# skit-ai/N-Best-ASR-Transformer

Measured on AMD Instinct MI355X. Metric: utterances/sec fine-tune (bert-base, seq128, n_best=5), higher is better.
Workload: dtype bf16

## Files before the change

include/nbest_hip.h:

```cpp
#ifndef NBEST_HIP_H
#define NBEST_HIP_H

#include <stddef.h>
#include <stdint.h>

#ifdef __cplusplus
extern "C" {
#endif

#define NBEST_ABI_VERSION 1

enum { NBEST_OK = 0, NBEST_ERR_ARG = -1, NBEST_ERR_SHAPE = -2, NBEST_ERR_DTYPE = -3, NBEST_ERR_ALIGN = -4,
       NBEST_ERR_LAUNCH = -5, NBEST_ERR_WORKSPACE = -6 };
enum { NBEST_F32 = 0, NBEST_BF16 = 1 };

typedef void* nbest_stream_t;

int nbest_version(void);
int nbest_last_error(char* buf, size_t n);

int nbest_embed_ln_fwd(const int64_t* ids, const int64_t* seg, const int64_t* pos, const void* word,
                       const void* type, const void* ptab, const float* gamma, const float* beta, void* out,
                       float* stats, int64_t M, int H, float eps, int dtype, float drop_p, uint64_t seed,
                       uint32_t drop_stream, nbest_stream_t stream);
// ... 176 lines not shown
} nbest_tensor_desc;
int nbest_bertadam_chunk(void);
int nbest_bertadam_step(float* p, float* g, float* m, float* v, void* p_lowp, const nbest_tensor_desc* descs,
                        int n_tensors, int n_blocks, float lr_mult, float b1, float b2, float eps,
                        float max_grad_norm, void* ws, size_t ws_bytes, nbest_stream_t stream);
int nbest_bertadam_norms(const float* g, const nbest_tensor_desc* descs, int n_tensors, int n_blocks, int blk_lo, int blk_hi,
                         float* partial, nbest_stream_t stream);
int nbest_bertadam_update(float* p, const float* g, float* m, float* v, void* p_lowp, const nbest_tensor_desc* descs,
                          int n_tensors, int n_blocks, int blk_lo, int blk_hi, const float* partial, float* coef,
                          float lr_mult, float b1, float b2, float eps, float max_grad_norm, nbest_stream_t stream);
enum { NBEST_ADAM_L2 = 0, NBEST_ADAMW = 1 };
int nbest_adam_clip_coef(const float* partial, int n_partial, float max_grad_norm, float* clip, nbest_stream_t stream);
int nbest_adam_update(int mode, float* p, const float* g, float* m, float* v, void* p_lowp, const nbest_tensor_desc* descs,
                      int n_tensors, int n_blocks, int blk_lo, int blk_hi, const float* clip, float lr_mult, float bc1,
                      float bc2_sqrt, double b1, double b2, float eps, nbest_stream_t stream);
int nbest_adam_step(int mode, float* p, float* g, float* m, float* v, void* p_lowp, const nbest_tensor_desc* descs,
                    int n_tensors, int n_blocks, float lr_mult, float bc1, float bc2_sqrt, double b1, double b2, float eps,
                    float max_grad_norm, void* ws, size_t ws_bytes, nbest_stream_t stream);
typedef struct nbest_matrix_desc {
  int64_t offset;
  int32_t rows, cols;
  int32_t tile_start, pad;
} nbest_matrix_desc;
#define NBEST_AMAX_TENSOR_WORDS 1024
int nbest_fp8_amax_fold(void* slots, void* out, int32_t n_tensors, nbest_stream_t stream);
int nbest_quantize_weights_fp8(const float* master, void* w8, void* w8t, const nbest_matrix_desc* descs, int n_matrices,
                               int n_tiles, float* inv_scale, void* ws, size_t ws_bytes, nbest_stream_t stream);
int nbest_transpose_weights(const void* src, void* dst, const nbest_matrix_desc* descs, int n_matrices, int n_tiles,
                            nbest_stream_t stream);
int nbest_pack_bn(int64_t N);
int nbest_pack_bn_fp8(int64_t N, int64_t K);
int nbest_pack_weights_fp8(const void* src, void* dst, const nbest_matrix_desc* descs, int n_matrices, int n_stages, nbest_stream_t stream);
int nbest_pack_weights(const void* src, void* dst, const nbest_matrix_desc* descs, int n_matrices, int n_stages, nbest_stream_t stream);
int nbest_cast_f32_to_bf16(const float* src, void* dst, int64_t n, nbest_stream_t stream);

typedef struct nbest_layer_offsets {
  int64_t wqkv, bqkv, wo, bo, ln1_g, ln1_b, w1, b1, w2, b2, ln2_g, ln2_b;
} nbest_layer_offsets;
typedef struct nbest_encoder_desc {
  int32_t dtype, B, S, H, L, heads, F;
  int32_t vocab, max_pos, n_types;
  float ln_eps, hidden_drop, attn_drop;
  int64_t word_pad_id, pos_pad_id;
  int64_t off_word, off_pos, off_type, off_emb_ln_g, off_emb_ln_b;
  const nbest_layer_offsets* layers_host;
  uint64_t seed;
  uint32_t drop_stream_base;
  int32_t wgrad_events_n;
  void** wgrad_events;
  const void* w8;
  const float* w8_inv_scale;
  const void* w8t;
  const uint32_t* gamax_prev;
  uint32_t* gamax_new;
  int32_t fp8_bwd;
  int32_t pad2;
  const void* wpk;
  const void* wpkt;
  const void* w8p;
  const void* w8tp;
  const int32_t* word_perm;
  const uint32_t* aamax_prev;
  uint32_t* aamax_new;
  int32_t fp8_act;
  int32_t pad4;
  int32_t first_trainable;
// ... 35 lines not shown
```

n-best-asr-transformer_amd/arena.py:

```python
import ctypes as C

import torch

from . import hipabi as hb
from .synth import encoder_param_shapes, head_param_shapes

ALIGN = 64

NO_DECAY = ("bias", "LayerNorm.bias", "LayerNorm.weight")


class Slot:
    __slots__ = ("name", "shape", "offset", "numel")

    def __init__(self, name, shape, offset):
        self.name, self.shape, self.offset = name, tuple(shape), offset
        n = 1
        for s in shape:
            n *= s
        self.numel = n


class ParamArena:
    def __init__(self, cfg, labels, device, compute_dtype=torch.bfloat16):
# ... 71 lines not shown
        self._pdescs = None
        if self.w16 is not None and self.device.type == "cuda":
            self.w16t = torch.zeros(self.total, dtype=torch.bfloat16, device=self.device)
            H, F = cfg.hidden_size, cfg.intermediate_size
            mats = []
            for o in self.layer_offsets:
                mats += [(o.wqkv, 3 * H, H), (o.wo, H, H), (o.w1, F, H), (o.w2, H, F)]
            arr = (hb.MatrixDesc * len(mats))()
            t = 0
            for i, (off, r, c) in enumerate(mats):
                arr[i].offset, arr[i].rows, arr[i].cols, arr[i].tile_start = off, r, c, t
                t += ((r + 63) // 64) * ((c + 63) // 64)
            self._tdescs = (torch.frombuffer(bytearray(bytes(arr)), dtype=torch.uint8).to(self.device), len(mats), t)
            self._pdescs = []
            for transposed in (False, True):
                sel = []
                for off, r, c in mats:
                    n, k = (c, r) if transposed else (r, c)
                    bn = hb.lib().nbest_pack_bn(n)
                    if not (bn > 0 and k % 32 == 0 and n % bn == 0):
                        sel = None
                        break
                    sel.append((off, n, k, bn))
                if sel is None:
                    self._pdescs = None
                    break
                parr = (hb.MatrixDesc * len(sel))()
                t = 0
                for i, (off, n, k, bn) in enumerate(sel):
                    parr[i].offset, parr[i].rows, parr[i].cols, parr[i].tile_start, parr[i].pad = off, n, k, t, bn
                    t += (n // bn) * (k // 32)
                self._pdescs.append((torch.frombuffer(bytearray(bytes(parr)), dtype=torch.uint8).to(self.device), len(sel), t))
            if self._pdescs is not None:
                self.wpk = torch.zeros(self.total, dtype=torch.bfloat16, device=self.device)
                self.wpkt = torch.zeros(self.total, dtype=torch.bfloat16, device=self.device)
        self._descs = None

    def view(self, buf, name):
        s = self.by_name[name]
        return buf[s.offset:s.offset + s.numel].view(s.shape)

    def heads_wb(self):
        R, H = self.labels.n_head_rows, self.cfg.hidden_size
        return self.p[self.off_wh:self.off_wh + R * H].view(R, H), self.p[self.off_bh:self.off_bh + R]

    def heads_grad_wb(self):
        R, H = self.labels.n_head_rows, self.cfg.hidden_size
        return self.g[self.off_wh:self.off_wh + R * H].view(R, H), self.g[self.off_bh:self.off_bh + R]

    @property
    def weights(self):
        return self.w16 if self.w16 is not None else self.p

    def refresh_compute_copy(self):
        if self.w16 is not None:
            hb.cast_bf16(self.p, self.w16)
        self.refresh_transposed()

    def refresh_transposed(self):
        if self.w16t is not None:
            if self.lazy_w16t:
                self.w16t_stale = True
            else:
                self.refresh_w16t()
        if self.w8 is not None:
            d, n, t = self._tdescs
            hb.check(hb.lib().nbest_quantize_weights_fp8(hb.ptr(self.p), hb.ptr(self.w8), hb.ptr(self.w8t), hb.ptr(d), n, t,
                                                         hb.ptr(self.w8_inv_scale), hb.ptr(self._w8_ws), self._w8_ws.numel(),
                                                         hb.stream_ptr()), "quantize_weights_fp8")
            if getattr(self, "w8p", None) is not None:
                for src, dst, (pd, pn, pt) in ((self.w8, self.w8p, self._p8descs[0]), (self.w8t, self.w8tp, self._p8descs[1])):
                    hb.check(hb.lib().nbest_pack_weights_fp8(hb.ptr(src), hb.ptr(dst), hb.ptr(pd), pn, pt, hb.stream_ptr()), "pack_weights_fp8")

    def refresh_w16t(self):
        d, n, t = self._tdescs
        hb.check(hb.lib().nbest_transpose_weights(hb.ptr(self.w16), hb.ptr(self.w16t), hb.ptr(d), n, t, hb.stream_ptr()),
                 "transpose_weights")
        self.w16t_stale = False
        if self.wpk is not None:
            for src, dst, (pd, pn, pt) in ((self.w16, self.wpk, self._pdescs[0]), (self.w16t, self.wpkt, self._pdescs[1])):
                hb.check(hb.lib().nbest_pack_weights(hb.ptr(src), hb.ptr(dst), hb.ptr(pd), pn, pt, hb.stream_ptr()), "pack_weights")

    def enable_fp8_forward(self):
        if self.w16t is None:
            raise RuntimeError("nbest_amd: the fp8 forward needs the bf16 path on a GPU")
        self.wpk = self.wpkt = None
        if self.w8 is None:
            n = self._tdescs[1]
            self.w8 = torch.zeros(self.total, dtype=torch.uint8, device=self.device)
            self.w8t = torch.zeros(self.total, dtype=torch.uint8, device=self.device)
            self.gamax = torch.zeros(n, dtype=torch.int32, device=self.device)
            self.gamax_slots = torch.zeros(n * hb.AMAX_TENSOR_WORDS, dtype=torch.int32, device=self.device)
            self.aamax = torch.zeros(n, dtype=torch.int32, device=self.device)
            self.aamax_slots = torch.zeros(n * hb.AMAX_TENSOR_WORDS, dtype=torch.int32, device=self.device)
            self.w8_inv_scale = torch.ones(n, dtype=torch.float32, device=self.device)
            self._w8_ws = torch.zeros(4 * n + 16, dtype=torch.uint8, device=self.device)
            H, F = self.cfg.hidden_size, self.cfg.intermediate_size
            mats = []
            for o in self.layer_offsets:
                mats += [(o.wqkv, 3 * H, H), (o.wo, H, H), (o.w1, F, H), (o.w2, H, F)]
            self._p8descs = []
            for transposed in (False, True):
                parr = (hb.MatrixDesc * len(mats))()
                t = 0
                for i, (off, r, c) in enumerate(mats):
                    nn, kk = (c, r) if transposed else (r, c)
                    bn = hb.lib().nbest_pack_bn_fp8(nn, kk)
                    if not (bn > 0 and kk % 64 == 0 and nn % bn == 0):
                        parr = None
                        break
                    parr[i].offset, parr[i].rows, parr[i].cols, parr[i].tile_start, parr[i].pad = off, nn, kk, t, bn
                    t += (nn // bn) * (kk // 64)
                if parr is None:
                    self._p8descs = None
# ... 63 lines not shown
```

n-best-asr-transformer_amd/csrc/gemm.hip:

```cpp
#include "common.h"

namespace {

__global__ __launch_bounds__(256) void splitk_reduce_kernel(const float* __restrict__ slab, float* __restrict__ C, int64_t MN,
                                                            int64_t N, int64_t ldc, int splits, int accumulate,
                                                            float* __restrict__ C2, int64_t m_split, int64_t ldc2) {
  for (int64_t i = ((int64_t)blockIdx.x * blockDim.x + threadIdx.x) * 4; i < MN; i += (int64_t)gridDim.x * blockDim.x * 4) {
    f32x4 s = *(const f32x4*)(slab + i);
    for (int z = 1; z < splits; ++z) s += *(const f32x4*)(slab + (int64_t)z * MN + i);
    const int64_t m = i / N, n = i - m * N;
    float* c = (m < m_split) ? C + m * ldc + n : C2 + (m - m_split) * ldc2 + n;
    if (accumulate) s += *(const f32x4*)c;
    *(f32x4*)c = s;
  }
}

int check_epilogue_operands(const nbest_gemm_args* a, int64_t ld_mult, uintptr_t align) {
  const int epi = a->epilogue;
  if (epi == NBEST_EPI_BIAS || epi == NBEST_EPI_BIAS_GELU || epi == NBEST_EPI_BIAS_DROP_RES)
    NB_CHECK(a->bias, NBEST_ERR_ARG, "gemm: epilogue %d needs bias", epi);
  if (epi == NBEST_EPI_BIAS_DROP_RES || epi == NBEST_EPI_RES)
    NB_CHECK(a->R && a->ldr % ld_mult == 0 && ((uintptr_t)a->R & (align - 1)) == 0, NBEST_ERR_ARG, "gemm: epilogue %d needs R", epi);
  if ((epi == NBEST_EPI_BIAS_GELU && a->U) || epi == NBEST_EPI_DGELU)
    NB_CHECK(a->U && a->ldu % ld_mult == 0 && ((uintptr_t)a->U & (align - 1)) == 0, NBEST_ERR_ARG, "gemm: epilogue %d needs U", epi);
// ... 47 lines not shown
  if (a->dtype == NBEST_F32) return (a->colsum_out && a->epilogue != NBEST_EPI_F32_SPLITK) ? nbest_rowred_ws_bytes(a->M, a->N) : 0;
  if (a->dtype != NBEST_BF16) return 0;
  const size_t w1 = nbest_gemm_bf16_ws_bytes(a), w2 = nbest_gemm_bf16_v2_ws_bytes(a);
  return w1 > w2 ? w1 : w2;
}

extern "C" int nbest_gemm(const nbest_gemm_args* a, nbest_stream_t stream) {
  NB_CHECK(a && a->A && a->B && a->C, NBEST_ERR_ARG, "gemm: null pointer");
  NB_CHECK(a->M > 0 && a->N > 0 && a->K > 0, NBEST_ERR_SHAPE, "gemm: bad shape %lld x %lld x %lld", (long long)a->M,
           (long long)a->N, (long long)a->K);
  if (a->dtype == NBEST_F32) {
    if (int rc = check_epilogue_operands(a, 1, 1)) return rc;
    if (int rc = nbest_gemm_f32(a, (hipStream_t)stream)) return rc;
    if (a->colsum_out && a->epilogue != NBEST_EPI_F32_SPLITK) {
      NB_CHECK(a->ws && a->ws_bytes >= nbest_rowred_ws_bytes(a->M, a->N), NBEST_ERR_WORKSPACE, "gemm(f32): column-sum workspace too small");
      return nbest_colsum(a->C, a->colsum_out, a->M, a->N, a->ldc, NBEST_F32, a->colsum_accumulate, a->ws, a->ws_bytes, stream);
    }
    return NBEST_OK;
  }
  if (a->dtype == NBEST_BF16) {
    if (int rc = check_bf16(a)) return rc;
    return nbest_gemm_bf16_v2_wins(a) ? nbest_gemm_bf16_v2(a, (hipStream_t)stream) : nbest_gemm_bf16(a, (hipStream_t)stream);
  }
  nbest_set_error("gemm: bad dtype %d", a->dtype);
  return NBEST_ERR_DTYPE;
}

extern "C" int nbest_pack_bn(int64_t N) { return nbest_pack_bn_internal(N); }
extern "C" int nbest_pack_weights(const void* src, void* dst, const nbest_matrix_desc* descs, int n_matrices, int n_stages,
                                  nbest_stream_t stream) {
  NB_CHECK(src && dst && descs && n_matrices > 0 && n_stages > 0 && src != dst, NBEST_ERR_ARG, "pack_weights: bad arguments");
  return nbest_pack_weights_bf16(src, dst, descs, n_matrices, n_stages, (hipStream_t)stream);
}

extern "C" size_t nbest_wgrad_pair_ws_bytes(const nbest_gemm_args* a, const nbest_gemm_args* b) {
  if (!a || !b) return 0;
  return nbest_wgrad_pair_bf16_ws_bytes(a, b);
}

extern "C" int nbest_wgrad_pair(const nbest_gemm_args* a, const nbest_gemm_args* b, nbest_stream_t stream) {
  NB_CHECK(a && b && a->A && a->B && a->C && b->A && b->B && b->C, NBEST_ERR_ARG, "wgrad_pair: null pointer");
  NB_CHECK(a->M > 0 && b->M > 0 && a->N > 0 && a->K > 0, NBEST_ERR_SHAPE, "wgrad_pair: bad shape");
  NB_CHECK(nbest_wgrad_pair_bf16_ws_bytes(a, b) > 0, NBEST_ERR_SHAPE,
           "wgrad_pair: needs two bf16 F32_SPLITK problems (trans_a = trans_b = 1) with equal N, K and accumulate, M1, M2, N multiples of 256 "
           "and at least 18 output tiles in all");
  if (int rc = check_bf16(a)) return rc;
  if (int rc = check_bf16(b)) return rc;
  return nbest_wgrad_pair_bf16(a, b, (hipStream_t)stream);
}

static int check_wgrad_table(const char* who, const nbest_gemm_args* problems, int n) {
  for (int i = 0; i < n; ++i) {
    const nbest_gemm_args* a = problems + i;
    NB_CHECK(a->A && a->B && a->C, NBEST_ERR_ARG, "%s: null pointer in problem %d", who, i);
    NB_CHECK(a->M > 0 && a->N > 0 && a->K > 0, NBEST_ERR_SHAPE, "%s: bad shape in problem %d", who, i);
    NB_CHECK(a->dtype == NBEST_BF16, NBEST_ERR_DTYPE, "%s: bf16 operands only", who);
    NB_CHECK(a->M % 256 == 0 && a->N % 256 == 0, NBEST_ERR_SHAPE, "%s: problem %d: %lld x %lld is not a multiple of the 256 x 256 tile", who, i,
             (long long)a->M, (long long)a->N);
    if (int rc = check_bf16(a)) return rc;
  }
  return NBEST_OK;
}

extern "C" int nbest_wgrad_group(const nbest_gemm_args* problems, int n, nbest_stream_t stream) {
  NB_CHECK(problems && n >= 1 && n <= 8, NBEST_ERR_ARG, "wgrad_group: needs 1 .. 8 problems");
  if (int rc = check_wgrad_table("wgrad_group", problems, n)) return rc;
// ... 10 lines not shown
```

n-best-asr-transformer_amd/csrc/gemm_bf16_v2.hip:

```cpp
#include "common.h"
#include <type_traits>

namespace {

constexpr int BK = 32;

struct GemmP2 {
  const bf16* A; const bf16* B; void* C; const float* bias; const bf16* R; bf16* U; float* slab; float* colpart;
  int64_t M, N, K, lda, ldb, ldc, ldr, ldu;
  int64_t k_per_split;
  int tiles_m, tiles_n, splits, accumulate;
  uint32_t a_bytes, b_bytes;
  uint32_t c_bytes, r_bytes, u_bytes;
  DropCfg drop;
  int stream_out;
  int gn;
  const bf16* A2; const bf16* B2;
  int64_t lda2, ldb2, m_split;
  uint32_t a2_bytes, b2_bytes;
  const bf16* Bp;
  uint32_t bp_bytes;
  int bp_bn;
};

// ... 793 lines not shown
constexpr int kMaxGroup = 16;
struct WgradProb {
  const bf16* A; const bf16* B; float* C;
  int64_t lda, ldb, ldc;
  uint32_t a_bytes, b_bytes;
  int tiles_m, tiles_n, gn, tile_start, tile_first;
};
struct WgradGroupP {
  WgradProb pr[kMaxGroup];
  int64_t K, k_pad;
  int n, accumulate;
};

template <int BM, int BN, int WM, int WN, int STAGES, bool TA, bool TB, int EPI>
__global__ __launch_bounds__(WM * WN * 64, 2) void gemm2_kernel_grouped(WgradGroupP g) {
  static_assert(BM == 256 && BN == 256 && TA && TB && EPI == NBEST_EPI_F32_SPLITK, "grouped launch: the 256 x 256 weight-gradient program only");
  const int id = xcd_remap(blockIdx.x, gridDim.x);
  WgradProb q = g.pr[0];
#pragma unroll
  for (int i = 1; i < kMaxGroup; ++i)
    if (i < g.n && id >= g.pr[i].tile_start) q = g.pr[i];
  GemmP2 p = {};
  p.A = q.A; p.B = q.B; p.C = q.C;
  p.M = (int64_t)q.tiles_m * 256; p.N = (int64_t)q.tiles_n * 256; p.K = g.K;
  p.lda = q.lda; p.ldb = q.ldb; p.ldc = q.ldc;
  p.k_per_split = g.k_pad;
  p.tiles_m = q.tiles_m; p.tiles_n = q.tiles_n; p.splits = 1; p.accumulate = g.accumulate;
  p.a_bytes = q.a_bytes; p.b_bytes = q.b_bytes;
  p.stream_out = 1;
  p.gn = q.gn;
  gemm2_body<BM, BN, WM, WN, STAGES, TA, TB, EPI>(p, id - q.tile_start + q.tile_first);
}

__global__ __launch_bounds__(256) void pack_b_kernel(const bf16* __restrict__ src, bf16* __restrict__ dst,
                                                     const nbest_matrix_desc* __restrict__ descs, int n) {
  int lo = 0, hi = n - 1;
  while (lo < hi) {
    const int mid = (lo + hi + 1) >> 1;
    if (descs[mid].tile_start <= (int)blockIdx.x) lo = mid; else hi = mid - 1;
  }
  const nbest_matrix_desc d = descs[lo];
  const int bn = d.pad, pw = (bn == 256) ? 128 : 96;
  const int nk = d.cols / BK, t = blockIdx.x - d.tile_start, tile_n = t / nk, kt = t - tile_n * nk;
  const bf16* s = src + d.offset + ((int64_t)tile_n * bn) * d.cols + (int64_t)kt * BK;
  bf16* o = dst + d.offset + ((int64_t)tile_n * nk + kt) * bn * BK;
  for (int p = threadIdx.x; p < bn * 4; p += blockDim.x) {
    const int row = p >> 2, slot = p & 3;
    const int kc = slot ^ ((-(row >> 2)) & 3);
    const int x = row % pw;
    const int grow = row - x + (pw / 16) * (x & 15) + (x >> 4);
    *(i32x4*)(o + (int64_t)p * 8) = *(const i32x4*)(s + (int64_t)grow * d.cols + kc * 8);
  }
}

struct Plan {
  int bm, bn, splits;
  int64_t kps;
};

static Plan make_plan(const nbest_gemm_args* a) {
  Plan pl;
  pl.bn = 128;
  const int64_t t256 = ((a->M + 255) / 256) * (a->N / 128);
  pl.bm = (!a->trans_a && t256 >= 1024) ? 256 : 128;
  const bool ok256 = (a->N % 256 == 0) && (!a->trans_a || a->M % 256 == 0);
  if (!a->trans_a && !a->trans_b && a->N % 256 == 0 &&
      [&] {
        const int64_t t = ((a->M + 255) / 256) * (a->N / 256);
        return t >= 1024 || (t >= 256 && (double)t / (double)(((t + 255) / 256) * 256) >= 0.85);
      }()) {
    pl.bm = 256; pl.bn = 256;
  } else if (a->trans_a && a->trans_b && a->epilogue == NBEST_EPI_F32_SPLITK && ok256 && (a->M / 256) * (a->N / 256) >= 18) {
    pl.bm = 256; pl.bn = 256;
  }
  {
    const bool epi192 = a->epilogue == NBEST_EPI_NONE || a->epilogue == NBEST_EPI_BIAS || a->epilogue == NBEST_EPI_BIAS_DROP_RES ||
                        a->epilogue == NBEST_EPI_RES;
    if (!a->trans_a && !a->trans_b && a->N % 192 == 0 && epi192) {
      const int64_t rows = (a->M + 255) / 256, t192 = rows * (a->N / 192);
      auto eff = [](int64_t t) { return (double)t / (double)(((t + 255) / 256) * 256); };
      const double e256 = (a->N % 256 == 0) ? eff(rows * (a->N / 256)) : 0.0;
      if (t192 >= 256 && 0.85 * eff(t192) > e256) { pl.bm = 256; pl.bn = 192; }
    }
    if (pl.bm == 256 && pl.bn == 192 && a->N % 384 == 0 && a->K % BK == 0) { pl.bm = 128; pl.bn = 384; }
    if (pl.bm == 256 && pl.bn == 256 && !a->trans_a && !a->trans_b && epi192 && a->N % 512 == 0 && a->N <= 2048 && a->K % BK == 0) { pl.bm = 128; pl.bn = 512; }
  }
  const int64_t tiles = ((a->M + pl.bm - 1) / pl.bm) * (a->N / pl.bn);
  const int64_t slots = (pl.bn >= 192) ? 256 : 512;
  pl.splits = 1;
  pl.kps = round_up(a->K, 64);
  if (a->epilogue == NBEST_EPI_F32_SPLITK) nb_splitk_plan(tiles, a->K, slots, (4 * slots + 4) / 5, &pl.splits, &pl.kps);
  return pl;
}

template <int BM, int BN, int WM, int WN, int STAGES, bool TA, bool TB>
static int launch2(const GemmP2& p, int epi, int grid, hipStream_t st) {
  constexpr int NT = WM * WN * 64;
  constexpr int lds_bytes = STAGES * (BM + BN) * BK * 2 + (((BN * 4) % NT) ? (NT / 64) * 1024 : 0);
#define L(E)                                                                                                        \
  case E:                                                                                                           \
    (void)hipFuncSetAttribute((const void*)gemm2_kernel<BM, BN, WM, WN, STAGES, TA, TB, E>, hipFuncAttributeMaxDynamicSharedMemorySize, lds_bytes); \
    gemm2_kernel<BM, BN, WM, WN, STAGES, TA, TB, E><<<grid, NT, lds_bytes, st>>>(p);                                 \
    break;
  if constexpr (BN / WN == 64) {
    if (epi == NBEST_EPI_F32_SPLITK) {
      switch (epi) { L(NBEST_EPI_F32_SPLITK) }
      NB_LAUNCH_CHECK();
// ... 181 lines not shown
    q.tiles_m = (int)(a->M / 256); q.tiles_n = (int)(a->N / 256);
    q.gn = (q.tiles_n > q.tiles_m && q.tiles_n % 3 == 0) ? 3 : q.tiles_n;
    q.tile_start = (int)tiles; q.tile_first = (int)f;
    tiles += c;
    NB_CHECK(tiles <= max_tiles, NBEST_ERR_ARG, "%s: more than %lld tiles in one launch", who, (long long)max_tiles);
  }
  constexpr int lds_bytes = 4 * (256 + 256) * BK * 2;
  const auto kernel = gemm2_kernel_grouped<256, 256, 2, 4, 4, true, true, NBEST_EPI_F32_SPLITK>;
  (void)hipFuncSetAttribute((const void*)kernel, hipFuncAttributeMaxDynamicSharedMemorySize, lds_bytes);
  kernel<<<(int)tiles, 512, lds_bytes, st>>>(g);
  NB_LAUNCH_CHECK();
  return NBEST_OK;
}

int nbest_wgrad_group_bf16(const nbest_gemm_args* pr, int n, hipStream_t st) {
  return wgrad_table_launch("wgrad_group", pr, nullptr, nullptr, n, 8, (int64_t)1 << 30, st);
}

int nbest_wgrad_window_bf16(const nbest_gemm_args* pr, const int32_t* first, const int32_t* count, int n, hipStream_t st) {
  return wgrad_table_launch("wgrad_window", pr, first, count, n, kMaxGroup, 256, st);
}

int nbest_pack_bn_internal(int64_t N) {
  if (N % 256 == 0 && N >= 1024) return 256;
  if (N % 192 == 0) return 192;
  return 0;
}

int nbest_pack_weights_bf16(const void* src, void* dst, const nbest_matrix_desc* descs, int n_matrices, int n_stages, hipStream_t st) {
  pack_b_kernel<<<n_stages, 256, 0, st>>>((const bf16*)src, (bf16*)dst, descs, n_matrices);
  NB_LAUNCH_CHECK();
  return NBEST_OK;
}
```

n-best-asr-transformer_amd/csrc/internal.h:

```cpp
#pragma once
#include <hip/hip_runtime_api.h>
#include <stddef.h>
#include <stdint.h>

#include "../../include/nbest_hip.h"

struct Fp8Grad;

void nbest_set_error(const char* fmt, ...);

int nbest_internal_layernorm_fwd8(const void* x, const float* gamma, const float* beta, void* y, void* y8, float* stats,
                                  int64_t M, int H, float eps, int dtype, nbest_stream_t stream, const uint32_t* a_prev, uint32_t* a_new);
int nbest_internal_layernorm_bwd8(const void* dy, const void* x, const float* stats, const float* gamma, void* dx,
                                  void* dx_drop, float* dgamma, float* dbeta, float* dbias, int64_t M, int H, int dtype,
                                  int accumulate, float drop_p, uint64_t seed, uint32_t drop_stream, void* ws,
                                  size_t ws_bytes, nbest_stream_t stream, Fp8Grad f8);
int nbest_internal_partial_rows_sum(const float* part, int nrows, int N, float* out, int accumulate, hipStream_t st);
void nbest_internal_rowred_batch_begin();
void nbest_internal_rowred_batch_abort();
int nbest_internal_rowred_batch_flush(hipStream_t st);

int nbest_internal_attention_fwd8(const void* qkv, const uint8_t* key_mask, void* ctx, void* ctx8, float* lse, int B, int S, int heads,
                                  int d, int dtype, float drop_p, uint64_t seed, uint32_t drop_stream, nbest_stream_t stream,
                                  uint32_t* keep, const uint32_t* a_prev, uint32_t* a_new);
int nbest_internal_attention_bwd8(const void* qkv, const uint8_t* key_mask, const void* ctx, const void* dctx, const float* lse,
                                  void* dqkv, float* dbias, int accumulate, void* ws, size_t ws_bytes, int B, int S, int heads,
                                  int d, int dtype, float drop_p, uint64_t seed, uint32_t drop_stream, nbest_stream_t stream, Fp8Grad f8,
                                  const uint32_t* keep);
size_t nbest_internal_attention_keep_bytes(int B, int S, int heads);
int nbest_attention_cls_fwd_internal(const void* q, int64_t ldq, const void* kv, int64_t ldkv, const uint8_t* key_mask, void* ctx,
                                     int64_t ldctx, int B, int S, int heads, int d, int dtype, nbest_stream_t stream);
int nbest_internal_attention_cls_probs(const void* q, int64_t ldq, const void* kv, int64_t ldkv, const uint8_t* key_mask, float* probs,
                                       int64_t ldp, int B, int S, int heads, int d, int dtype, nbest_stream_t stream);

void nb_splitk_plan(int64_t tiles, int64_t K, int64_t slots, int64_t min_blocks, int* splits, int64_t* k_per_split);
int nbest_internal_splitk_reduce(const float* slab, float* C, int64_t M, int64_t N, int64_t ldc, int splits, int accumulate,
                                 float* C2, int64_t m_split, int64_t ldc2, hipStream_t st);

int nbest_gemm_f32(const nbest_gemm_args* a, hipStream_t st);
size_t nbest_gemm_bf16_ws_bytes(const nbest_gemm_args* a);
int nbest_gemm_bf16(const nbest_gemm_args* a, hipStream_t st);
size_t nbest_gemm_bf16_v2_ws_bytes(const nbest_gemm_args* a);
int nbest_gemm_bf16_v2(const nbest_gemm_args* a, hipStream_t st);
bool nbest_gemm_bf16_v2_wins(const nbest_gemm_args* a);
size_t nbest_wgrad_pair_bf16_ws_bytes(const nbest_gemm_args* a, const nbest_gemm_args* b);
int nbest_wgrad_pair_bf16(const nbest_gemm_args* a, const nbest_gemm_args* b, hipStream_t st);
int nbest_wgrad_group_bf16(const nbest_gemm_args* problems, int n, hipStream_t st);
int nbest_wgrad_window_bf16(const nbest_gemm_args* problems, const int32_t* tile_first, const int32_t* tile_count, int n, hipStream_t st);
int nbest_pack_bn_internal(int64_t N);
int nbest_pack_weights_bf16(const void* src, void* dst, const nbest_matrix_desc* descs, int n_matrices, int n_stages, hipStream_t st);

int nbest_internal_amax_bf16(const void* x, int64_t n, uint32_t* out, hipStream_t st);
int nbest_internal_cast_bf16_to_fp8(const void* src, void* dst, int64_t n, const uint32_t* a_prev, uint32_t* a_new, hipStream_t st);
```

n-best-asr-transformer_amd/hipabi.py:

```python
import ctypes as C
import os

import torch

_HERE = os.path.dirname(os.path.abspath(__file__))
LIB_PATH = os.environ.get("NBEST_LIB") or os.path.join(_HERE, "csrc", "libnbest_hip.so")

F32, BF16 = 0, 1
ADAM_L2, ADAMW = 0, 1
EPI_NONE, EPI_BIAS, EPI_BIAS_GELU, EPI_BIAS_DROP_RES, EPI_DGELU, EPI_RES, EPI_F32_SPLITK = range(7)

EXPORTS = [
    "nbest_version", "nbest_last_error", "nbest_embed_ln_fwd", "nbest_embed_ln_bwd", "nbest_embed_bwd_ws_bytes", "nbest_rows_gather", "nbest_rows_zero", "nbest_rows_add",
    "nbest_gemm_ws_bytes", "nbest_gemm", "nbest_wgrad_pair_ws_bytes", "nbest_wgrad_pair", "nbest_wgrad_group", "nbest_wgrad_window", "nbest_pack_bn", "nbest_pack_weights", "nbest_pack_bn_fp8", "nbest_pack_weights_fp8", "nbest_attention_fwd", "nbest_attention_bwd", "nbest_attention_bwd_ws_bytes", "nbest_attention_keep_bytes", "nbest_attention_fwd_keep", "nbest_attention_bwd_keep", "nbest_layernorm_fwd",
    "nbest_layernorm_bwd", "nbest_rowred_ws_bytes", "nbest_colsum", "nbest_heads_ws_bytes", "nbest_stc_heads",
    "nbest_stc_heads_vjp", "nbest_cls_mse", "nbest_cls_grad_scatter", "nbest_stc_decode", "nbest_stream_stamp", "nbest_fp8_amax_fold", "nbest_bertadam_chunk", "nbest_bertadam_step", "nbest_bertadam_norms", "nbest_bertadam_update",
    "nbest_adam_clip_coef", "nbest_adam_update", "nbest_adam_step",
    "nbest_cast_f32_to_bf16", "nbest_transpose_weights", "nbest_encoder_act_bytes", "nbest_encoder_ws_bytes", "nbest_encoder_wgrad_launches_per_layer", "nbest_encoder_wgrad_plan", "nbest_encoder_forward",
    "nbest_encoder_backward", "nbest_gemm_fp8", "nbest_gemm_fp8_ws_bytes", "nbest_wgrad_fp8", "nbest_wgrad_fp8_ws_bytes", "nbest_wgrad_fp8_pair", "nbest_wgrad_fp8_pair_ws_bytes", "nbest_cast_bf16_to_fp8", "nbest_quantize_weights_fp8",
    "nbest_attention_cls_fwd", "nbest_encoder_infer_ws_bytes", "nbest_encoder_infer",
    "nbest_attention_probs", "nbest_attention_cls_probs", "nbest_encoder_act_view", "nbest_encoder_infer_attn",
    "nbest_embed_ln_fwd_interp", "nbest_embed_attrib",
    "nbest_head_gate_fwd", "nbest_head_gate_bwd",
]


class GemmArgs(C.Structure):
    _fields_ = [("A", C.c_void_p), ("B", C.c_void_p), ("C", C.c_void_p), ("bias", C.c_void_p), ("R", C.c_void_p),
                ("U", C.c_void_p), ("ws", C.c_void_p), ("ws_bytes", C.c_size_t),
                ("M", C.c_int64), ("N", C.c_int64), ("K", C.c_int64),
                ("lda", C.c_int64), ("ldb", C.c_int64), ("ldc", C.c_int64), ("ldr", C.c_int64), ("ldu", C.c_int64),
                ("trans_a", C.c_int32), ("trans_b", C.c_int32), ("epilogue", C.c_int32), ("dtype", C.c_int32),
                ("accumulate", C.c_int32), ("drop_p", C.c_float), ("drop_stream", C.c_uint32), ("seed", C.c_uint64),
                ("colsum_out", C.c_void_p), ("colsum_accumulate", C.c_int32), ("flags", C.c_int32),
                ("B_packed", C.c_void_p), ("b_pack_bn", C.c_int32), ("pad_", C.c_int32)]


class GemmFp8Args(C.Structure):
    _fields_ = [("A", C.c_void_p), ("B", C.c_void_p), ("C", C.c_void_p), ("bias", C.c_void_p), ("R", C.c_void_p), ("U", C.c_void_p),
                ("C8", C.c_void_p), ("M", C.c_int64), ("N", C.c_int64), ("K", C.c_int64),
                ("lda", C.c_int64), ("ldb", C.c_int64), ("ldc", C.c_int64), ("ldr", C.c_int64), ("ldu", C.c_int64), ("ldc8", C.c_int64),
                ("epilogue", C.c_int32), ("out_scale", C.c_float), ("drop_p", C.c_float), ("drop_stream", C.c_uint32), ("seed", C.c_uint64),
                ("out_scale_dev", C.c_void_p), ("a_amax", C.c_void_p), ("c8_amax_prev", C.c_void_p), ("c8_amax_new", C.c_void_p),
                ("colsum_out", C.c_void_p), ("colsum_accumulate", C.c_int32), ("pad", C.c_int32), ("ws", C.c_void_p), ("ws_bytes", C.c_size_t),
                ("B_packed", C.c_void_p), ("b_pack_bn", C.c_int32), ("pad3", C.c_int32)]


# ... 80 lines not shown
        L.nbest_attention_keep_bytes.argtypes = [i32, i32, i32]
        L.nbest_attention_fwd_keep.argtypes = [vp] * 4 + [i32] * 5 + [f32, u64, u32, vp, vp]
        L.nbest_attention_bwd_keep.argtypes = [vp] * 7 + [i32, vp, sz] + [i32] * 5 + [f32, u64, u32, vp, vp]
        L.nbest_layernorm_fwd.argtypes = [vp] * 5 + [i64, i32, f32, i32, vp]
        L.nbest_layernorm_bwd.argtypes = [vp] * 9 + [i64, i32, i32, i32, f32, u64, u32, vp, sz, vp]
        L.nbest_colsum.argtypes = [vp, vp, i64, i64, i64, i32, i32, vp, sz, vp]
        L.nbest_stc_heads.argtypes = [vp, i64, vp, vp, C.POINTER(LabelSpaceC)] + [vp] * 8 + [i32] * 5 + [f32, u64, u32, vp, sz, vp]
        L.nbest_stc_heads_vjp.argtypes = [vp, C.POINTER(LabelSpaceC)] + [vp] * 8 + [i32, i32, i32, f32, u64, u32, vp, sz, vp]
        L.nbest_cls_mse.argtypes = [vp, i64, vp, i64, vp, vp, vp, i32, i32, i32, f32, vp]
        L.nbest_cls_grad_scatter.argtypes = [vp, vp, i32, i32, i32, i32, vp]
        L.nbest_stc_decode.argtypes = [vp, vp, C.POINTER(LabelSpaceC), vp, vp, i32, vp]
        L.nbest_stream_stamp.argtypes = [vp, i32, vp]
        L.nbest_fp8_amax_fold.argtypes = [vp, vp, i32, vp]
        L.nbest_bertadam_step.argtypes = [vp] * 6 + [i32, i32, f32, f32, f32, f32, f32, vp, sz, vp]
        L.nbest_bertadam_norms.argtypes = [vp, vp, i32, i32, i32, i32, vp, vp]
        L.nbest_bertadam_update.argtypes = [vp] * 6 + [i32, i32, i32, i32, vp, vp, f32, f32, f32, f32, f32, vp]
        L.nbest_adam_clip_coef.argtypes = [vp, i32, f32, vp, vp]
        f64 = C.c_double
        L.nbest_adam_update.argtypes = [i32] + [vp] * 6 + [i32, i32, i32, i32, vp, f32, f32, f32, f64, f64, f32, vp]
        L.nbest_adam_step.argtypes = [i32] + [vp] * 6 + [i32, i32, f32, f32, f32, f64, f64, f32, f32, vp, sz, vp]
        L.nbest_cast_f32_to_bf16.argtypes = [vp, vp, i64, vp]
        L.nbest_encoder_forward.argtypes = [C.POINTER(EncoderDesc)] + [vp] * 7 + [sz, vp, sz, C.POINTER(C.c_void_p), vp]
        L.nbest_encoder_infer_ws_bytes.argtypes = [C.POINTER(EncoderDesc)]
        L.nbest_encoder_infer.argtypes = [C.POINTER(EncoderDesc)] + [vp] * 7 + [sz, vp, vp]
        L.nbest_attention_cls_fwd.argtypes = [vp, i64, vp, i64, vp, vp, i64, i32, i32, i32, i32, i32, vp]
        L.nbest_encoder_infer_attn.argtypes = [C.POINTER(EncoderDesc)] + [vp] * 7 + [sz, vp, vp, vp]
        L.nbest_encoder_act_view.argtypes = [C.POINTER(EncoderDesc), vp, i32, C.POINTER(C.c_void_p), C.POINTER(C.c_void_p)]
        L.nbest_attention_probs.argtypes = [vp] * 4 + [i32] * 5 + [vp]
        L.nbest_attention_cls_probs.argtypes = [vp, i64, vp, i64, vp, vp, i64, i32, i32, i32, i32, i32, vp]
        L.nbest_encoder_backward.argtypes = [C.POINTER(EncoderDesc)] + [vp] * 9 + [sz, vp, vp, sz, i32, i32, i32, i32, vp]
        L.nbest_transpose_weights.argtypes = [vp, vp, vp, i32, i32, vp]
        L.nbest_pack_bn.argtypes = [i64]
        L.nbest_pack_weights.argtypes = [vp, vp, vp, i32, i32, vp]
        L.nbest_pack_bn_fp8.argtypes = [i64, i64]
        L.nbest_pack_weights_fp8.argtypes = [vp, vp, vp, i32, i32, vp]
        L.nbest_gemm_fp8.argtypes = [C.POINTER(GemmFp8Args), vp]
        L.nbest_cast_bf16_to_fp8.argtypes = [vp, vp, i64, vp]
        L.nbest_wgrad_fp8_ws_bytes.restype = C.c_size_t
        L.nbest_wgrad_fp8_ws_bytes.argtypes = [i64, i64, i64]
        L.nbest_wgrad_fp8.argtypes = [vp, vp, vp, i64, i64, i64, i64, i64, i64, vp, vp, i32, vp, sz, vp]
        L.nbest_wgrad_fp8_pair_ws_bytes.restype = C.c_size_t
        L.nbest_wgrad_fp8_pair_ws_bytes.argtypes = [i64, i64, i64, i64]
        L.nbest_wgrad_fp8_pair.argtypes = [vp, vp, vp, i64, i64, i64, i64, vp, vp, vp, vp, vp, i64, i64, i64, i64, vp, vp, i64, i64, i32, vp, sz, vp]
        L.nbest_quantize_weights_fp8.argtypes = [vp, vp, vp, vp, i32, i32, vp, vp, sz, vp]
        L.nbest_gemm_fp8_ws_bytes.restype = C.c_size_t
        L.nbest_gemm_fp8_ws_bytes.argtypes = [C.POINTER(GemmFp8Args)]
        L.nbest_last_error.argtypes = [C.c_char_p, sz]
        _lib = L
    return _lib


def last_error():
    buf = C.create_string_buffer(512)
    lib().nbest_last_error(buf, 512)
    return buf.value.decode(errors="replace")


def check(rc, what):
    if rc != 0:
        raise RuntimeError("nbest_hip %s failed (%d): %s" % (what, rc, last_error()))


def stream_ptr():
    return C.c_void_p(torch.cuda.current_stream().cuda_stream)


# ... 518 lines not shown
```

Baseline: 12880.

## Fuse weight transpose and both packings into one LDS-tiled kernel

Replaces the three separate passes that rebuild the weight images after each optimizer step (transpose to w16t, pack w16, pack w16t) with a single kernel. Each block loads one weight tile into LDS once, writes the packed image, transposes the tile in registers and LDS, then writes both the transposed arena and its packed image. This removes repeated global reads of the source and the extra launches. It also changes the GEMM plan so that untransposed 128x128 non-split-K GEMMs whose K is not a multiple of 64 use BM=256. The costs are a large dynamic-LDS kernel with per-block matrix lookup and new swizzle logic whose correctness depends on the tile shapes.

After: 12960, median of 6. Within noise of the previous version (+0.6%).

```diff
diff --git a/include/nbest_hip.h b/include/nbest_hip.h
--- a/include/nbest_hip.h
+++ b/include/nbest_hip.h
@@ -232,6 +232,9 @@
 int nbest_pack_bn_fp8(int64_t N, int64_t K);
 int nbest_pack_weights_fp8(const void* src, void* dst, const nbest_matrix_desc* descs, int n_matrices, int n_stages, nbest_stream_t stream);
 int nbest_pack_weights(const void* src, void* dst, const nbest_matrix_desc* descs, int n_matrices, int n_stages, nbest_stream_t stream);
+int nbest_refresh_weight_images(const void* w16, void* w16t, void* wpk, void* wpkt, const nbest_matrix_desc* tdescs,
+                                const nbest_matrix_desc* pdescs, const nbest_matrix_desc* pdescs_t, int n_matrices, int n_tiles, int max_bn,
+                                nbest_stream_t stream);
 int nbest_cast_f32_to_bf16(const float* src, void* dst, int64_t n, nbest_stream_t stream);
 
 typedef struct nbest_layer_offsets {
diff --git a/n-best-asr-transformer_amd/arena.py b/n-best-asr-transformer_amd/arena.py
--- a/n-best-asr-transformer_amd/arena.py
+++ b/n-best-asr-transformer_amd/arena.py
@@ -127,6 +127,9 @@
                     t += (n // bn) * (k // 32)
                 self._pdescs.append((torch.frombuffer(bytearray(bytes(parr)), dtype=torch.uint8).to(self.device), len(sel), t))
             if self._pdescs is not None:
+                bns = [(hb.lib().nbest_pack_bn(r), hb.lib().nbest_pack_bn(c)) for _, r, c in mats]
+                self._img_tiles = sum((r // br) * (c // bc) for (_, r, c), (br, bc) in zip(mats, bns))
+                self._img_max_bn = max(max(b) for b in bns)
                 self.wpk = torch.zeros(self.total, dtype=torch.bfloat16, device=self.device)
                 self.wpkt = torch.zeros(self.total, dtype=torch.bfloat16, device=self.device)
         self._descs = None
@@ -169,12 +172,15 @@
 
     def refresh_w16t(self):
         d, n, t = self._tdescs
+        if self.wpk is not None:
+            hb.check(hb.lib().nbest_refresh_weight_images(hb.ptr(self.w16), hb.ptr(self.w16t), hb.ptr(self.wpk), hb.ptr(self.wpkt), hb.ptr(d),
+                                                          hb.ptr(self._pdescs[0][0]), hb.ptr(self._pdescs[1][0]), n, self._img_tiles,
+                                                          self._img_max_bn, hb.stream_ptr()), "refresh_weight_images")
+            self.w16t_stale = False
+            return
         hb.check(hb.lib().nbest_transpose_weights(hb.ptr(self.w16), hb.ptr(self.w16t), hb.ptr(d), n, t, hb.stream_ptr()),
                  "transpose_weights")
         self.w16t_stale = False
-        if self.wpk is not None:
-            for src, dst, (pd, pn, pt) in ((self.w16, self.wpk, self._pdescs[0]), (self.w16t, self.wpkt, self._pdescs[1])):
-                hb.check(hb.lib().nbest_pack_weights(hb.ptr(src), hb.ptr(dst), hb.ptr(pd), pn, pt, hb.stream_ptr()), "pack_weights")
 
     def enable_fp8_forward(self):
         if self.w16t is None:
diff --git a/n-best-asr-transformer_amd/csrc/gemm.hip b/n-best-asr-transformer_amd/csrc/gemm.hip
--- a/n-best-asr-transformer_amd/csrc/gemm.hip
+++ b/n-best-asr-transformer_amd/csrc/gemm.hip
@@ -103,6 +103,15 @@
   NB_CHECK(src && dst && descs && n_matrices > 0 && n_stages > 0 && src != dst, NBEST_ERR_ARG, "pack_weights: bad arguments");
   return nbest_pack_weights_bf16(src, dst, descs, n_matrices, n_stages, (hipStream_t)stream);
 }
+extern "C" int nbest_refresh_weight_images(const void* w16, void* w16t, void* wpk, void* wpkt, const nbest_matrix_desc* tdescs,
+                                           const nbest_matrix_desc* pdescs, const nbest_matrix_desc* pdescs_t, int n_matrices, int n_tiles,
+                                           int max_bn, nbest_stream_t stream) {
+  NB_CHECK(w16 && w16t && wpk && wpkt && tdescs && pdescs && pdescs_t && n_matrices > 0 && n_tiles > 0, NBEST_ERR_ARG,
+           "refresh_weight_images: bad arguments");
+  NB_CHECK(w16 != w16t && w16 != wpk && w16 != wpkt && w16t != wpk && w16t != wpkt && wpk != wpkt, NBEST_ERR_ARG,
+           "refresh_weight_images: the four arenas must be distinct");
+  return nbest_refresh_weight_images_bf16(w16, w16t, wpk, wpkt, tdescs, pdescs, pdescs_t, n_matrices, n_tiles, max_bn, (hipStream_t)stream);
+}
 
 extern "C" size_t nbest_wgrad_pair_ws_bytes(const nbest_gemm_args* a, const nbest_gemm_args* b) {
   if (!a || !b) return 0;
diff --git a/n-best-asr-transformer_amd/csrc/gemm_bf16_v2.hip b/n-best-asr-transformer_amd/csrc/gemm_bf16_v2.hip
--- a/n-best-asr-transformer_amd/csrc/gemm_bf16_v2.hip
+++ b/n-best-asr-transformer_amd/csrc/gemm_bf16_v2.hip
@@ -849,6 +849,15 @@
   gemm2_body<BM, BN, WM, WN, STAGES, TA, TB, EPI>(p, id - q.tile_start + q.tile_first);
 }
 
+__host__ __device__ constexpr int pack_pw(int bn) { return bn == 256 ? 128 : 96; }
+struct PackSrc { int grow, kc; };
+__device__ __forceinline__ PackSrc pack_chunk_src(int p, int pw) {
+  const int row = p >> 2, slot = p & 3;
+  const int kc = slot ^ ((-(row >> 2)) & 3);
+  const int x = row % pw;
+  return PackSrc{row - x + (pw / 16) * (x & 15) + (x >> 4), kc};
+}
+
 __global__ __launch_bounds__(256) void pack_b_kernel(const bf16* __restrict__ src, bf16* __restrict__ dst,
                                                      const nbest_matrix_desc* __restrict__ descs, int n) {
   int lo = 0, hi = n - 1;
@@ -857,17 +866,133 @@
     if (descs[mid].tile_start <= (int)blockIdx.x) lo = mid; else hi = mid - 1;
   }
   const nbest_matrix_desc d = descs[lo];
-  const int bn = d.pad, pw = (bn == 256) ? 128 : 96;
+  const int bn = d.pad, pw = pack_pw(bn);
   const int nk = d.cols / BK, t = blockIdx.x - d.tile_start, tile_n = t / nk, kt = t - tile_n * nk;
   const bf16* s = src + d.offset + ((int64_t)tile_n * bn) * d.cols + (int64_t)kt * BK;
   bf16* o = dst + d.offset + ((int64_t)tile_n * nk + kt) * bn * BK;
   for (int p = threadIdx.x; p < bn * 4; p += blockDim.x) {
-    const int row = p >> 2, slot = p & 3;
-    const int kc = slot ^ ((-(row >> 2)) & 3);
-    const int x = row % pw;
-    const int grow = row - x + (pw / 16) * (x & 15) + (x >> 4);
-    *(i32x4*)(o + (int64_t)p * 8) = *(const i32x4*)(s + (int64_t)grow * d.cols + kc * 8);
-  }
+    const PackSrc c = pack_chunk_src(p, pw);
+    *(i32x4*)(o + (int64_t)p * 8) = *(const i32x4*)(s + (int64_t)c.grow * d.cols + c.kc * 8);
+  }
+}
+
+constexpr int kImgNT = 512, kImgMaxMats = 1024;
+
+template <int NCH>
+__device__ __forceinline__ int img_src_chunk(int r, int k) { return r * NCH + (k + r) % NCH; }
+template <int NCH>
+__device__ __forceinline__ int img_tr_chunk(int c, int k) { return c * NCH + (k + c + (c >> 3)) % NCH; }
+
+template <int TR, int TC>
+__device__ __forceinline__ void weight_images_tile(const bf16* __restrict__ s, bf16* __restrict__ o_t, bf16* __restrict__ o_pk,
+                                                   bf16* __restrict__ o_pkt, int R, int C, int rt, int ct, i32x4* lds, int tid) {
+  constexpr int NCH_C = TC / 8, NCH_R = TR / 8, TOTAL = TR * TC / 8, NI = TOTAL / kImgNT;
+  static_assert(TOTAL % kImgNT == 0, "whole rounds of 16-byte chunks");
+  const int64_t r0 = (int64_t)rt * TR, c0 = (int64_t)ct * TC;
+  {
+    i32x4 v[NI];
+#pragma unroll
+    for (int i = 0; i < NI; ++i) {
+      const int ch = i * kImgNT + tid, r = ch / NCH_C, k = ch % NCH_C;
+      v[i] = *(const i32x4*)(s + (r0 + r) * C + c0 + k * 8);
+    }
+#pragma unroll
+    for (int i = 0; i < NI; ++i) {
+      const int ch = i * kImgNT + tid, r = ch / NCH_C, k = ch % NCH_C;
+      lds[img_src_chunk<NCH_C>(r, k)] = v[i];
+    }
+  }
+  __syncthreads();
+  {
+    bf16* o = o_pk + ((int64_t)rt * (C / BK) + (int64_t)ct * (TC / BK)) * (TR * BK);
+#pragma unroll
+    for (int i = 0; i < NI; ++i) {
+      const int g = i * kImgNT + tid, j = g / (TR * 4), p = g % (TR * 4);
+      const PackSrc c = pack_chunk_src(p, pack_pw(TR));
+      *(i32x4*)(o + (int64_t)g * 8) = lds[img_src_chunk<NCH_C>(c.grow, j * 4 + c.kc)];
+    }
+  }
+  {
+    constexpr int NB = NCH_R * NCH_C, NBI = (NB + kImgNT - 1) / kImgNT;
+    uint32_t in[NBI][8][4];
+#pragma unroll
+    for (int it = 0; it < NBI; ++it) {
+      const int b = it * kImgNT + tid, rb = b / NCH_C, cb = b % NCH_C;
+      if (b < NB) {
+#pragma unroll
+        for (int i = 0; i < 8; ++i) {
+          const i32x4 x = lds[img_src_chunk<NCH_C>(rb * 8 + i, cb)];
+          in[it][i][0] = (uint32_t)x[0]; in[it][i][1] = (uint32_t)x[1]; in[it][i][2] = (uint32_t)x[2]; in[it][i][3] = (uint32_t)x[3];
+        }
+      }
+    }
+    __syncthreads();
+#pragma unroll
+    for (int it = 0; it < NBI; ++it) {
+      const int b = it * kImgNT + tid, rb = b / NCH_C, cb = b % NCH_C;
+      if (b < NB) {
+#pragma unroll
+        for (int j = 0; j < 8; ++j) {
+          i32x4 x;
+#pragma unroll
+          for (int w = 0; w < 4; ++w) {
+            const uint32_t a = in[it][2 * w][j >> 1], bb = in[it][2 * w + 1][j >> 1];
+            x[w] = (int)((j & 1) ? ((a >> 16) | (bb & 0xFFFF0000u)) : ((a & 0xFFFFu) | (bb << 16)));
+          }
+          lds[img_tr_chunk<NCH_R>(cb * 8 + j, rb)] = x;
+        }
+      }
+    }
+  }
+  __syncthreads();
+  {
+    bf16* o = o_pkt + ((int64_t)ct * (R / BK) + (int64_t)rt * (TR / BK)) * (TC * BK);
+#pragma unroll
+    for (int i = 0; i < NI; ++i) {
+      const int g = i * kImgNT + tid, c = g / NCH_R, k = g % NCH_R;
+      *(i32x4*)(o_t + (c0 + c) * R + r0 + k * 8) = lds[img_tr_chunk<NCH_R>(c, k)];
+    }
+#pragma unroll
+    for (int i = 0; i < NI; ++i) {
+      const int g = i * kImgNT + tid, j = g / (TC * 4), p = g % (TC * 4);
+      const PackSrc c = pack_chunk_src(p, pack_pw(TC));
+      *(i32x4*)(o + (int64_t)g * 8) = lds[img_tr_chunk<NCH_R>(c.grow, j * 4 + c.kc)];
+    }
+  }
+}
+
+__global__ __launch_bounds__(kImgNT) void weight_images_kernel(const bf16* __restrict__ src, bf16* __restrict__ w16t, bf16* __restrict__ wpk,
+                                                               bf16* __restrict__ wpkt, const nbest_matrix_desc* __restrict__ td,
+                                                               const nbest_matrix_desc* __restrict__ pf,
+                                                               const nbest_matrix_desc* __restrict__ pt, int n, int lds_bytes) {
+  extern __shared__ __attribute__((aligned(16))) char img_lds[];
+  __shared__ int cnt[kImgMaxMats], found[2];
+  const int tid = threadIdx.x;
+  for (int i = tid; i < n; i += kImgNT) {
+    const int bf = pf[i].pad, bt = pt[i].pad;
+    cnt[i] = (bf > 0 && bt > 0) ? (td[i].rows / bf) * (td[i].cols / bt) : 0;
+  }
+  if (tid == 0) found[0] = -1;
+  __syncthreads();
+  for (int i = tid; i < n; i += kImgNT) {
+    int start = 0;
+    for (int u = 0; u < i; ++u) start += cnt[u];
+    if ((int)blockIdx.x >= start && (int)blockIdx.x < start + cnt[i]) { found[0] = i; found[1] = start; }
+  }
+  __syncthreads();
+  const int m = found[0];
+  if (m < 0) return;
+  const nbest_matrix_desc d = td[m];
+  const int bf = pf[m].pad, bt = pt[m].pad;
+  if (bf * bt * 2 > lds_bytes) return;
+  const int t = blockIdx.x - found[1], tiles_c = d.cols / bt, rt = t / tiles_c, ct = t - rt * tiles_c;
+  const bf16* s = src + d.offset;
+  bf16 *o_t = w16t + d.offset, *o_pk = wpk + d.offset, *o_pkt = wpkt + d.offset;
+  i32x4* lds = (i32x4*)img_lds;
+  if (bf == 192 && bt == 192) weight_images_tile<192, 192>(s, o_t, o_pk, o_pkt, d.rows, d.cols, rt, ct, lds, tid);
+  else if (bf == 256 && bt == 256) weight_images_tile<256, 256>(s, o_t, o_pk, o_pkt, d.rows, d.cols, rt, ct, lds, tid);
+  else if (bf == 192 && bt == 256) weight_images_tile<192, 256>(s, o_t, o_pk, o_pkt, d.rows, d.cols, rt, ct, lds, tid);
+  else if (bf == 256 && bt == 192) weight_images_tile<256, 192>(s, o_t, o_pk, o_pkt, d.rows, d.cols, rt, ct, lds, tid);
 }
 
 struct Plan {
@@ -890,6 +1015,8 @@
   } else if (a->trans_a && a->trans_b && a->epilogue == NBEST_EPI_F32_SPLITK && ok256 && (a->M / 256) * (a->N / 256) >= 18) {
     pl.bm = 256; pl.bn = 256;
   }
+  if (pl.bm == 128 && pl.bn == 128 && !a->trans_a && !a->trans_b && a->epilogue != NBEST_EPI_F32_SPLITK && a->K % 64 != 0 && a->K % BK == 0)
+    pl.bm = 256;
   {
     const bool epi192 = a->epilogue == NBEST_EPI_NONE || a->epilogue == NBEST_EPI_BIAS || a->epilogue == NBEST_EPI_BIAS_DROP_RES ||
                         a->epilogue == NBEST_EPI_RES;
@@ -1137,3 +1264,16 @@
   NB_LAUNCH_CHECK();
   return NBEST_OK;
 }
+
+int nbest_refresh_weight_images_bf16(const void* w16, void* w16t, void* wpk, void* wpkt, const nbest_matrix_desc* tdescs,
+                                     const nbest_matrix_desc* pdescs, const nbest_matrix_desc* pdescs_t, int n_matrices, int n_tiles, int max_bn,
+                                     hipStream_t st) {
+  NB_CHECK(n_matrices <= kImgMaxMats, NBEST_ERR_ARG, "refresh_weight_images: more than %d matrices", kImgMaxMats);
+  NB_CHECK(max_bn == 192 || max_bn == 256, NBEST_ERR_ARG, "refresh_weight_images: max_bn %d is no packing width", max_bn);
+  const int lds_bytes = max_bn * max_bn * 2;
+  (void)hipFuncSetAttribute((const void*)weight_images_kernel, hipFuncAttributeMaxDynamicSharedMemorySize, lds_bytes);
+  weight_images_kernel<<<n_tiles, kImgNT, lds_bytes, st>>>((const bf16*)w16, (bf16*)w16t, (bf16*)wpk, (bf16*)wpkt, tdescs, pdescs, pdescs_t,
+                                                           n_matrices, lds_bytes);
+  NB_LAUNCH_CHECK();
+  return NBEST_OK;
+}
diff --git a/n-best-asr-transformer_amd/csrc/internal.h b/n-best-asr-transformer_amd/csrc/internal.h
--- a/n-best-asr-transformer_amd/csrc/internal.h
+++ b/n-best-asr-transformer_amd/csrc/internal.h
@@ -49,6 +49,9 @@
 int nbest_wgrad_window_bf16(const nbest_gemm_args* problems, const int32_t* tile_first, const int32_t* tile_count, int n, hipStream_t st);
 int nbest_pack_bn_internal(int64_t N);
 int nbest_pack_weights_bf16(const void* src, void* dst, const nbest_matrix_desc* descs, int n_matrices, int n_stages, hipStream_t st);
+int nbest_refresh_weight_images_bf16(const void* w16, void* w16t, void* wpk, void* wpkt, const nbest_matrix_desc* tdescs,
+                                     const nbest_matrix_desc* pdescs, const nbest_matrix_desc* pdescs_t, int n_matrices, int n_tiles, int max_bn,
+                                     hipStream_t st);
 
 int nbest_internal_amax_bf16(const void* x, int64_t n, uint32_t* out, hipStream_t st);
 int nbest_internal_cast_bf16_to_fp8(const void* src, void* dst, int64_t n, const uint32_t* a_prev, uint32_t* a_new, hipStream_t st);
diff --git a/n-best-asr-transformer_amd/hipabi.py b/n-best-asr-transformer_amd/hipabi.py
--- a/n-best-asr-transformer_amd/hipabi.py
+++ b/n-best-asr-transformer_amd/hipabi.py
@@ -12,7 +12,7 @@
 
 EXPORTS = [
     "nbest_version", "nbest_last_error", "nbest_embed_ln_fwd", "nbest_embed_ln_bwd", "nbest_embed_bwd_ws_bytes", "nbest_rows_gather", "nbest_rows_zero", "nbest_rows_add",
-    "nbest_gemm_ws_bytes", "nbest_gemm", "nbest_wgrad_pair_ws_bytes", "nbest_wgrad_pair", "nbest_wgrad_group", "nbest_wgrad_window", "nbest_pack_bn", "nbest_pack_weights", "nbest_pack_bn_fp8", "nbest_pack_weights_fp8", "nbest_attention_fwd", "nbest_attention_bwd", "nbest_attention_bwd_ws_bytes", "nbest_attention_keep_bytes", "nbest_attention_fwd_keep", "nbest_attention_bwd_keep", "nbest_layernorm_fwd",
+    "nbest_gemm_ws_bytes", "nbest_gemm", "nbest_wgrad_pair_ws_bytes", "nbest_wgrad_pair", "nbest_wgrad_group", "nbest_wgrad_window", "nbest_pack_bn", "nbest_pack_weights", "nbest_refresh_weight_images", "nbest_pack_bn_fp8", "nbest_pack_weights_fp8", "nbest_attention_fwd", "nbest_attention_bwd", "nbest_attention_bwd_ws_bytes", "nbest_attention_keep_bytes", "nbest_attention_fwd_keep", "nbest_attention_bwd_keep", "nbest_layernorm_fwd",
     "nbest_layernorm_bwd", "nbest_rowred_ws_bytes", "nbest_colsum", "nbest_heads_ws_bytes", "nbest_stc_heads",
     "nbest_stc_heads_vjp", "nbest_cls_mse", "nbest_cls_grad_scatter", "nbest_stc_decode", "nbest_stream_stamp", "nbest_fp8_amax_fold", "nbest_bertadam_chunk", "nbest_bertadam_step", "nbest_bertadam_norms", "nbest_bertadam_update",
     "nbest_adam_clip_coef", "nbest_adam_update", "nbest_adam_step",
@@ -159,6 +159,7 @@
         L.nbest_transpose_weights.argtypes = [vp, vp, vp, i32, i32, vp]
         L.nbest_pack_bn.argtypes = [i64]
         L.nbest_pack_weights.argtypes = [vp, vp, vp, i32, i32, vp]
+        L.nbest_refresh_weight_images.argtypes = [vp, vp, vp, vp, vp, vp, vp, i32, i32, i32, vp]
         L.nbest_pack_bn_fp8.argtypes = [i64, i64]
         L.nbest_pack_weights_fp8.argtypes = [vp, vp, vp, i32, i32, vp]
         L.nbest_gemm_fp8.argtypes = [C.POINTER(GemmFp8Args), vp]
```
